# GAMES-UChile/mogptk

Hardware: AMD Instinct MI355X
Metric: log-marginal-likelihood+grad evals/sec, MOSM C=4 N=8192; 1/2/4/8 GPU (higher is better)
Workload: dtype f64

## Files before the change

include/mogp_hip.h:

```cpp
#ifndef MOGP_HIP_H
#define MOGP_HIP_H

#include <stdint.h>

#ifdef __cplusplus
extern "C" {
#endif

#define MOGP_OK            0
#define MOGP_EINVAL       -1
#define MOGP_EHIP         -2
#define MOGP_ENOTPD       -3
#define MOGP_ENONFINITE   -4
#define MOGP_ENODEVICE    -5

#define MOGP_TERM_WIDTH(D) (2 + 3 * (D))
#define MOGP_MOMENT_WIDTH(D) (2 + 3 * (D))

typedef struct mogp_ctx mogp_ctx;
typedef struct mogp_model mogp_model;

const char* mogp_version(void);
const char* mogp_last_error(void);
int  mogp_device_count(void);
// ... 108 lines not shown
int  mogp_model_fetch(mogp_model* m, int which, double* out);

int  mogp_snelson_eval(mogp_model* m, int64_t M, const double* Z, const double* noise_var, double jitter, const double* kff_diag, int flags,
                       double* lml, double* mom_uu, double* mom_uf, double* gZ, double* trGA, double* hsum, double* jitter_abs, int64_t* info);
int  mogp_snelson_predict(mogp_model* m, int64_t M, const double* Z, const double* noise_var, double jitter, const double* kff_diag,
                          const double* kss_diag, int64_t S, const double* Xs, double* mu, double* var, int64_t* info);
int  mogp_snelson_eval_sharded(mogp_model* m, int64_t M, const double* Z, const double* noise_var, double jitter, const double* kff_diag,
                               int flags, double* lml, double* mom_uu, double* mom_uf, double* gZ, double* trGA, double* hsum,
                               double* jitter_abs, int64_t* info);
int  mogp_snelson_predict_sharded(mogp_model* m, int64_t M, const double* Z, const double* noise_var, double jitter, const double* kff_diag,
                                  const double* kss_diag, int64_t S, const double* Xs, double* mu, double* var, int64_t* info);

int  mogp_svgp_forward(mogp_model* m, int64_t M, const double* Z, const double* q_mu, const double* q_sqrt, double jitter,
                       const double* kff_diag, int dense, int64_t S, const double* Xs, const double* kss_diag,
                       double* mu, double* var, double* jitter_abs, int64_t* info);
int  mogp_svgp_backward(mogp_model* m, const double* e, const double* f, double* mom_uu, double* mom_uf, double* gZ, double* trGA,
                        double* g_qmu, double* g_qsqrt);
int  mogp_svgp_backward_sharded(mogp_model* m, const double* e, const double* f, double* mom_uu, double* mom_uf, double* gZ, double* trGA,
                                double* g_qmu, double* g_qsqrt);

int  mogp_oa_forward(mogp_model* m, const double* q_nu, const double* q_lambda, double* mu, double* var, double* kl, int64_t* info);
int  mogp_oa_backward(mogp_model* m, const double* e, const double* f, double* moments, double* g_nu, double* g_lambda);
int  mogp_oa_predict(mogp_model* m, const double* q_nu, const double* q_lambda, const double* kss_diag, int64_t S, const double* Xs,
                     int full, double* mu, double* var, int64_t* info);

int  mogp_sparse_predict_cov(mogp_model* m, int64_t S, double* cov);

int  mogp_mosm_terms(int C, int Q, int D, const double* w, const double* mu, const double* v, const double* th, const double* ph,
                     double twopi, double phase_scale, double* table);
int  mogp_mosm_terms_backward(int C, int Q, int D, const double* w, const double* mu, const double* v, const double* th, const double* ph,
                              double twopi, double phase_scale, const double* gtable, double* gw, double* gmu, double* gv, double* gth,
                              double* gph);

#ifdef __cplusplus
}
#endif
#endif
```

mogptk_amd/_lib.py:

```python
import atexit
import ctypes
import os
import threading
import weakref
import numpy as np

_HERE = os.path.dirname(os.path.abspath(__file__))
LIB_PATH = os.environ.get("MOGP_LIB_PATH") or os.path.join(_HERE, "csrc", "libmogp_hip.so")

MOGP_OK, MOGP_EINVAL, MOGP_EHIP, MOGP_ENOTPD, MOGP_ENONFINITE, MOGP_ENODEVICE = 0, -1, -2, -3, -4, -5
MOGP_EVAL_GRAD = 1
COMM_ID_BYTES = 128
ALLGATHER_CB = ctypes.CFUNCTYPE(ctypes.c_int, ctypes.c_void_p, ctypes.c_void_p, ctypes.c_void_p, ctypes.c_int64)
ALLREDUCE_CB = ctypes.CFUNCTYPE(ctypes.c_int, ctypes.c_void_p, ctypes.c_void_p, ctypes.c_int64)
ST_GRAM, ST_POTRF, ST_TRTRI, ST_LAUUM, ST_SOLVE, ST_MOMENTS, ST_TOTAL, ST_GEMM_KERNEL, ST_GRAM_KERNEL, ST_MOMENT_KERNEL, ST_COUNT = range(11)

_lib = None
_lock = threading.RLock()
_ctx = {}
_live = weakref.WeakSet()

c_dp = ctypes.POINTER(ctypes.c_double)
c_i64p = ctypes.POINTER(ctypes.c_int64)
c_ip = ctypes.POINTER(ctypes.c_int)
# ... 60 lines not shown
    "mogp_shard_alpha": (ctypes.c_int, [ctypes.c_void_p, ctypes.POINTER(ctypes.c_void_p), c_i64p]),
    "mogp_shard_finish": (ctypes.c_int, [ctypes.c_void_p, c_dp, c_dp, c_dp, c_i64p]),
    "mogp_dev_copy": (ctypes.c_int, [ctypes.c_void_p, ctypes.c_void_p, ctypes.c_int64, ctypes.c_int]),
    "mogp_set_profiling": (ctypes.c_int, [ctypes.c_void_p, ctypes.c_int]),
    "mogp_stage_ms": (ctypes.c_int, [ctypes.c_void_p, c_dp, c_i64p, c_dp]),
    "mogp_model_fetch": (ctypes.c_int, [ctypes.c_void_p, ctypes.c_int, c_dp]),
    "mogp_model_schedule": (ctypes.c_int, [ctypes.c_void_p, ctypes.POINTER(ctypes.c_int)]),
    "mogp_model_flow_replay": (ctypes.c_int, [ctypes.c_void_p, ctypes.c_int]),
    "mogp_model_flow_diag": (ctypes.c_int, [ctypes.c_void_p, ctypes.POINTER(ctypes.c_uint)]),
    "mogp_flow_plan": (ctypes.c_int, [ctypes.c_int, c_i64p, ctypes.c_int64, c_i64p]),
    "mogp_flow_plan_rhs": (ctypes.c_int, [ctypes.c_int, ctypes.c_int, c_i64p, ctypes.c_int64, ctypes.POINTER(ctypes.c_int64)]),
    "mogp_flow_trace": (ctypes.c_int, [ctypes.c_void_p, c_i64p, ctypes.c_int64, c_i64p]),
    "mogp_snelson_eval": (ctypes.c_int, [ctypes.c_void_p, ctypes.c_int64, c_dp, c_dp, ctypes.c_double, c_dp, ctypes.c_int,
                                         ctypes.POINTER(ctypes.c_double), c_dp, c_dp, c_dp, ctypes.POINTER(ctypes.c_double), c_dp,
                                         ctypes.POINTER(ctypes.c_double), c_i64p]),
    "mogp_snelson_predict": (ctypes.c_int, [ctypes.c_void_p, ctypes.c_int64, c_dp, c_dp, ctypes.c_double, c_dp, c_dp, ctypes.c_int64, c_dp,
                                            c_dp, c_dp, c_i64p]),
    "mogp_snelson_eval_sharded": (ctypes.c_int, [ctypes.c_void_p, ctypes.c_int64, c_dp, c_dp, ctypes.c_double, c_dp, ctypes.c_int,
                                         ctypes.POINTER(ctypes.c_double), c_dp, c_dp, c_dp, ctypes.POINTER(ctypes.c_double), c_dp,
                                         ctypes.POINTER(ctypes.c_double), c_i64p]),
    "mogp_snelson_predict_sharded": (ctypes.c_int, [ctypes.c_void_p, ctypes.c_int64, c_dp, c_dp, ctypes.c_double, c_dp, c_dp, ctypes.c_int64, c_dp,
                                            c_dp, c_dp, c_i64p]),
    "mogp_svgp_forward": (ctypes.c_int, [ctypes.c_void_p, ctypes.c_int64, c_dp, c_dp, c_dp, ctypes.c_double, c_dp, ctypes.c_int, ctypes.c_int64,
                                         c_dp, c_dp, c_dp, c_dp, ctypes.POINTER(ctypes.c_double), c_i64p]),
    "mogp_svgp_backward": (ctypes.c_int, [ctypes.c_void_p, c_dp, c_dp, c_dp, c_dp, c_dp, ctypes.POINTER(ctypes.c_double), c_dp, c_dp]),
    "mogp_svgp_backward_sharded": (ctypes.c_int, [ctypes.c_void_p, c_dp, c_dp, c_dp, c_dp, c_dp, ctypes.POINTER(ctypes.c_double), c_dp, c_dp]),
    "mogp_oa_forward": (ctypes.c_int, [ctypes.c_void_p, c_dp, c_dp, c_dp, c_dp, ctypes.POINTER(ctypes.c_double), c_i64p]),
    "mogp_oa_backward": (ctypes.c_int, [ctypes.c_void_p, c_dp, c_dp, c_dp, c_dp, c_dp]),
    "mogp_oa_predict": (ctypes.c_int, [ctypes.c_void_p, c_dp, c_dp, c_dp, ctypes.c_int64, c_dp, ctypes.c_int, c_dp, c_dp, c_i64p]),
    "mogp_sparse_predict_cov": (ctypes.c_int, [ctypes.c_void_p, ctypes.c_int64, c_dp]),
    "mogp_mosm_terms": (ctypes.c_int, [ctypes.c_int, ctypes.c_int, ctypes.c_int, c_dp, c_dp, c_dp, c_dp, c_dp, ctypes.c_double, ctypes.c_double, c_dp]),
    "mogp_mosm_terms_backward": (ctypes.c_int, [ctypes.c_int, ctypes.c_int, ctypes.c_int, c_dp, c_dp, c_dp, c_dp, c_dp, ctypes.c_double,
                                                ctypes.c_double, c_dp, c_dp, c_dp, c_dp, c_dp, c_dp]),
}


class MogpError(RuntimeError):
    def __init__(self, code, message, info=0):
        super().__init__(message)
        self.code = code
        self.info = info


def lib():
    global _lib
    with _lock:
        if _lib is None:
            if not os.path.exists(LIB_PATH):
                raise ImportError(
                    "libmogp_hip.so not found at %s: build it with `python __graft_entry__.py` "
                    "(hipcc --offload-arch=gfx950).  mogptk_amd has no CPU fallback." % LIB_PATH)
            l = ctypes.CDLL(LIB_PATH)
            for name, (res, args) in SIGNATURES.items():
                fn = getattr(l, name)
                fn.restype = res
                fn.argtypes = args
            _lib = l
    return _lib


def _dp(a):
    return None if a is None else a.ctypes.data_as(c_dp)


def _f64(a):
    return None if a is None else np.ascontiguousarray(a, dtype=np.float64)
# ... 40 lines not shown
    M2 = M1 if X2 is None else X2.shape[0]
    out = np.empty((M1, M2), dtype=np.float64)
    if kind is not None:
        kind = np.ascontiguousarray(kind, dtype=np.int32)
        shape = _f64(shape)
        assert kind.shape == table.shape[:3] and shape.shape == table.shape[:3]
        check(lib().mogp_gram_kinds(context(device), C, D, T, int(table.shape[3]), _dp(table), _ip(kind), _dp(shape), M1, _dp(X1),
                                    0 if X2 is None else M2, _dp(X2), _dp(out)))
        return out
    check(lib().mogp_gram_ex(context(device), C, D, T, int(table.shape[3]), _dp(table), M1, _dp(X1),
                             0 if X2 is None else M2, _dp(X2), _dp(out)))
    return out


def shutdown():
    with _lock:
        for h in list(_live):
            try:
                h.close()
            except Exception:
                pass
        if _lib is not None:
            for c in list(_ctx.values()):
                try:
                    _lib.mogp_ctx_destroy(c)
                except Exception:
                    pass
        _ctx.clear()


atexit.register(shutdown)


class ExactHandle:

    def __init__(self, device, X, y, C):
        X = _f64(X)
        y = _f64(np.asarray(y).reshape(-1))
        self.N = X.shape[0]
        self.D = X.shape[1] - 1
        self.C = C
        self.device = device
        h = ctypes.c_void_p()
        self._h = ctypes.c_void_p()
        check(lib().mogp_model_create(context(device), self.N, self.D, C, _dp(X), _dp(y), ctypes.byref(h)))
        self._h = h
        _live.add(self)

    def close(self):
        if getattr(self, "_h", None) is not None and self._h.value is not None:
            lib().mogp_model_destroy(self._h)
            self._h = ctypes.c_void_p()

    def __del__(self):
        try:
            self.close()
        except Exception:
            pass

    def set_y(self, y):
        y = _f64(np.asarray(y).reshape(-1))
        check(lib().mogp_model_set_y(self._h, _dp(y)))

    def set_mean(self, coef):
        if coef is None:
            check(lib().mogp_model_set_mean(self._h, None))
# ... 13 lines not shown
        self.T = table.shape[2]
        self.W = int(table.shape[3])
        check(lib().mogp_model_set_terms_ex(self._h, self.T, self.W, _dp(table)))

    def set_kinds(self, kind, shape):
        if kind is None:
            check(lib().mogp_model_set_kinds(self._h, self.T, None, None))
            return
        kind = np.ascontiguousarray(kind, dtype=np.int32)
        shape = _f64(shape)
        assert kind.shape == (self.C, self.C, self.T) and shape.shape == kind.shape
        check(lib().mogp_model_set_kinds(self._h, self.T, _ip(kind), _dp(shape)))

    def set_point_diag(self, kdiag):
        check(lib().mogp_model_set_point_diag(self._h, _dp(_f64(kdiag))))

    def eval(self, noise_var, jitter, grad=True, data_var=None):
        noise_var = _f64(noise_var)
        data_var = _f64(data_var)
        from .gpr.config import config as _cfg
        comm = getattr(_cfg, "comm", None)
        if grad and comm is not None and (comm.world > 1 or comm.force):
            if getattr(comm, "native", False):
                return self.eval_sharded(noise_var, jitter, data_var)
            from . import dist as _dist
            return _dist.sharded_eval(self, comm, noise_var, jitter, data_var)
        lml, trG, jit, info = ctypes.c_double(), ctypes.c_double(), ctypes.c_double(), ctypes.c_int64(0)
        moments, diagG = self._grad_outputs(grad)
        code = lib().mogp_exact_eval(self._h, _dp(noise_var), _dp(data_var), float(jitter),
                                     MOGP_EVAL_GRAD if grad else 0, ctypes.byref(lml), _dp(moments), _dp(diagG),
                                     ctypes.byref(trG), ctypes.byref(jit), ctypes.byref(info))
        check(code, info.value)
        return dict(lml=lml.value, moments=moments, diagG=diagG, trG=trG.value, jitter_abs=jit.value)

    def _grad_outputs(self, grad=True):
        C = self.C
        return (np.zeros((C * (C + 1) // 2, self.T, self.W)), np.zeros(C)) if grad else (None, None)

    def _held_out(self, key, entry, noise_var, jitter, grad, data_var, *score_args):
        noise_var = _f64(noise_var)
        data_var = _f64(data_var)
        score, trG, jit, info = ctypes.c_double(), ctypes.c_double(), ctypes.c_double(), ctypes.c_int64(0)
        mu, var = np.empty(self.N), np.empty(self.N)
        moments, diagG = self._grad_outputs(grad)
        code = entry(self._h, _dp(noise_var), _dp(data_var), float(jitter), MOGP_EVAL_GRAD if grad else 0, *score_args, ctypes.byref(score),
                     _dp(mu), _dp(var), _dp(moments), _dp(diagG), ctypes.byref(trG), ctypes.byref(jit), ctypes.byref(info))
        check(code, info.value)
        return {key: score.value, "mu": mu, "var": var, "moments": moments, "diagG": diagG, "trG": trG.value, "jitter_abs": jit.value}

    def loo(self, noise_var, jitter, grad=True, data_var=None):
        return self._held_out("loo", lib().mogp_exact_loo, noise_var, jitter, grad, data_var)

    def cv(self, noise_var, jitter, fold, nfolds, grad=True, data_var=None):
        fold = np.ascontiguousarray(fold, dtype=np.int32)
        if fold.shape != (self.N,):
            raise ValueError("fold must hold one label per training point")
        return self._held_out("cv", lib().mogp_exact_cv, noise_var, jitter, grad, data_var, fold.ctypes.data_as(ctypes.POINTER(ctypes.c_int32)), int(nfolds))

    def loo_bytes(self):
        b = ctypes.c_int64(0)
        check(lib().mogp_model_loo_bytes(self._h, ctypes.byref(b)))
        return int(b.value)

    def eval_sharded(self, noise_var, jitter, data_var=None):
        lml, trG, jit, info = ctypes.c_double(), ctypes.c_double(), ctypes.c_double(), ctypes.c_int64(0)
        moments, diagG = self._grad_outputs()
# ... 252 lines not shown
```

mogptk_amd/gpr/config.py:

```python
import numpy as np


class Config:
    dtype = np.float64
    device = 0
    positive_minimum = 1e-8
    comm = None
    accurate_fallback = True


config = Config()


def use_double_precision():
    config.dtype = np.float64


def use_single_precision():
    config.dtype = np.float32


def use_half_precision():
    raise NotImplementedError("half precision is not on the MI355X exact-GP path")


def use_gpu(n=None):
    from .._lib import lib
    count = lib().mogp_device_count()
    if count <= 0:
        print("HIP device is not available")
    elif n is not None and (not isinstance(n, int) or n < 0 or count <= n):
        print("HIP GPU '%s' is not available" % (n,))
    else:
        config.device = 0 if n is None else n


def use_hip(n=None):
    use_gpu(n)


def use_cpu(n=None):
# ... 17 lines not shown
```

mogptk_amd/gpr/model.py:

```python
import sys
import numpy as np
from contextlib import contextmanager
from math import erf, sqrt

from .config import config
from .parameter import Parameter, ParameterHolder
from .kernel import Kernel, MulKernel, ChangePointsKernel, terms_cache, KIND_TIMES, KIND_MASK, KIND_DOT, KIND_GATE, KIND_WDOT, group_diag_grad
from .likelihood import Likelihood, GaussianLikelihood
from .mean import Mean


class CholeskyException(Exception):

    def __init__(self, message, K, model):
        self.message = message
        self.K = K
        self.model = model

    def __str__(self):
        return self.message


def _to_array(X):
    if hasattr(X, "detach"):
        X = X.detach().cpu().numpy()
    return np.array(X, dtype=config.dtype)


def _leaf_kernels(kernel):
    subs = getattr(kernel, "kernels", None)
    if not subs or isinstance(kernel, (MulKernel, ChangePointsKernel)):
        return [kernel]
    return [leaf for k in subs for leaf in _leaf_kernels(k)]


def _enveloped(table, D):
    return table.shape[3] > 2 + 3 * D


def _channel_counts(Xk, C):
    return np.bincount(Xk[:, 0].astype(np.int64), minlength=C).astype(np.float64)


def _lml_constant(X):
    return 0.5 * X.shape[0] * np.log(2.0 * np.pi)


_PAIR_INDEX = {}


def _pair_index(C, lower):
    key = (C, lower)
    if key not in _PAIR_INDEX:
        _PAIR_INDEX[key] = np.tril_indices(C) if lower else tuple(np.divmod(np.arange(C * C), C))
    return _PAIR_INDEX[key]


def _gtable_from_moments(table, mom, D, lower=True, kind=None):
    C, T = table.shape[0], table.shape[2]
    gt = np.zeros((C, C, T, table.shape[3]))
    ii, jj = _pair_index(C, lower)
    tb = table[ii, jj]
    A = tb[..., 0]
    V = tb[..., 2:2 + D]
    M = tb[..., 2 + D:2 + 2 * D]
    m0, m4 = mom[..., 0], mom[..., 1]
    m1, m2, m3 = mom[..., 2:2 + D], mom[..., 2 + D:2 + 2 * D], mom[..., 2 + 2 * D:2 + 3 * D]
    g = np.empty_like(tb)
    g[..., 0] = m0
    g[..., 1] = -2.0 * np.pi * A * m4
    g[..., 2:2 + D] = -0.5 * A[..., None] * m1
    g[..., 2 + D:2 + 2 * D] = -2.0 * np.pi * A[..., None] * m3
    g[..., 2 + 2 * D:2 + 3 * D] = -V * A[..., None] * m2 - 2.0 * np.pi * M * (A * m4)[..., None]
    if tb.shape[-1] > 2 + 3 * D:
        Lv = tb[..., 2 + 3 * D:2 + 4 * D]
        g[..., 2 + 3 * D:2 + 4 * D] = -0.5 * A[..., None] * mom[..., 2 + 3 * D:2 + 4 * D]
        g[..., 2 + 4 * D:2 + 5 * D] = Lv * A[..., None] * mom[..., 2 + 4 * D:2 + 5 * D]
    if kind is not None:
# ... 368 lines not shown
                if np.any(taken):
                    raise ValueError("folds %d and %d overlap (point %d): folds are disjoint" % (labels[ind][taken][0], f, ind[taken][0]))
                labels[ind] = f
        if F == 0:
            raise ValueError("no folds: at least one point must be held out")
        sizes = np.bincount(labels[labels >= 0], minlength=F)
        for f in range(F):
            if sizes[f] == 0:
                raise ValueError("fold %d is empty" % f)
            if sizes[f] > self.FOLD_MAX:
                raise ValueError("fold %d holds %d points: the limit is %d points per fold, larger folds are not on the device"
                                 % (f, sizes[f], self.FOLD_MAX))
        return labels.astype(np.int32), F

    def _eval(self, grad, score="lml", folds=None):
        if score == "loo":
            self._refuse_sharded_loo()
        elif score == "cv":
            self._refuse_sharded_loo("leave-fold-out cross-validation")
            labels, F = self._fold_labels(folds)
        h, table, D = self._push_terms()
        with self._cholesky_guard():
            if score == "cv":
                run = lambda: h.cv(self._noise_var(), self.jitter, labels, F, grad=grad, data_var=self.data_variance)
            else:
                call = h.loo if score == "loo" else h.eval
                run = lambda: call(self._noise_var(), self.jitter, grad=grad, data_var=self.data_variance)
            res = run()
            again = self._check_conditioning(h, run) if grad or score != "lml" else None
            return (res if again is None else again), table, D

    CONDITION_WARN = 1e5

    def _check_conditioning(self, h, redo):
        if not hasattr(h, "condition_estimate"):
            return None
        est = h.condition_estimate()
        if est != est:
            return None
        accurate = getattr(h, "accurate_mode", False)
        if not accurate and est > self.CONDITION_WARN:
            fallback = getattr(config, "accurate_fallback", True) and hasattr(h, "set_accurate")
            if not getattr(self, "_cond_warned", False):
                self._cond_warned = True
                import warnings
                warnings.warn("the kernel matrix plus noise is ill-conditioned (cond >= %.1e from the Cholesky factor's diagonal): beyond ~1e6 - 1e7 the "
                              "fast schedules' LML and gradients leave a backward-stable factorisation's by more than 1e-9 / 1e-5 (at 1e8: ~1e-7 / ~1e-4); %s"
                              % (est, "evaluating in the backward-stable form from here on (about two and a half times slower)" if fallback
                                 else "a larger noise variance or jitter brings it back"), RuntimeWarning, stacklevel=5)
            if fallback:
                h.set_accurate(True)
                h.accurate_mode = True
                return redo()
        elif accurate and est < 0.1 * self.CONDITION_WARN:
            h.set_accurate(False)
            h.accurate_mode = False
        return None

    def log_marginal_likelihood(self):
        res, _, _ = self._eval(grad=False)
        return config.dtype(res["lml"])

    def _loss_impl(self, score="lml", folds=None):
        self.zero_grad(set_to_none=True)
        res, table, D = self._eval(grad=True, score=score, folds=folds)
        counts = self._train_counts()
        jit_rel = self.jitter * res["trG"] / self.X.shape[0]

        point_kinds = getattr(self._handle, "point_kinds", None)
        gt = _gtable_from_moments(table, res["moments"], D, lower=True, kind=point_kinds)
        if _enveloped(table, D) or point_kinds is not None:
            gt += jit_rel * self.kernel._point_diag_table_grad(table, self.kernel._kernel_format(self.X), D)
        else:
            kind = getattr(self._handle, "group_kinds", None)
            if kind is not None:
                for i in range(table.shape[0]):
                    gt[i, i, :, 0] += jit_rel * counts[i] * group_diag_grad(table[i, i, :, 0], kind[i, i])
            else:
                for i in range(table.shape[0]):
                    gt[i, i, :, 0] += jit_rel * counts[i]
        self.kernel._table_backward(-gt)

        self._noise_backward(res["diagG"] + jit_rel * counts)
        self._mean_backward(self._handle)
        return config.dtype(-res[score] - self.log_prior())

    def loo(self):
        res, _, _ = self._eval(grad=False, score="loo")
        return self._held_out(res)

    def _held_out(self, res):
        mu = res["mu"].reshape(-1, 1)
        if self.mean is not None and not (self._trainable_mean() and self._mean_affine()[0] is not None):
            mu = self._add_mean(mu, self.X)
        return mu.astype(config.dtype, copy=False), res["var"].reshape(-1, 1).astype(config.dtype, copy=False)

# ... 429 lines not shown
```

mogptk_amd/gpr/multioutput.py:

```python
import ctypes

import numpy as np

from .config import config
from .parameter import Parameter, _STRUCTURE_EPOCH
from .kernel import Kernel, MultiOutputKernel, term_width, cached_terms, KIND_TIMES, KIND_MASK, KIND_DOT, GROUP_MAX, group_slices

PI = np.pi


def _accumulate(p, gconstrained):
    p.accumulate_grad(gconstrained)


class IndependentMultiOutputKernel(MultiOutputKernel):

    def __init__(self, *kernels, output_dims=None):
        if output_dims is None:
            output_dims = len(kernels)
        super().__init__(output_dims)
        self.kernels = self._check_kernels(kernels, output_dims)
        self.input_dims = self.kernels[0].input_dims

    def __getitem__(self, key):
# ... 55 lines not shown
        super().__init__(output_dims, input_dims, active_dims)
        self.input_dims = input_dims
        self.weight = Parameter(np.ones((output_dims, Q)), lower=config.positive_minimum)
        self.mean = Parameter(np.zeros((output_dims, Q, input_dims)), lower=config.positive_minimum)
        self.variance = Parameter(np.ones((output_dims, Q, input_dims)), lower=config.positive_minimum)
        self.delay = Parameter(np.zeros((output_dims, Q, input_dims)))
        self.phase = Parameter(np.zeros((output_dims, Q)))
        if output_dims == 1:
            self.delay.train = False
            self.phase.train = False
        self.twopi = np.power(2.0 * np.pi, float(self.input_dims) / 2.0)

    _phase_scale = 1.0

    def _values(self):
        return self.weight(), self.mean(), self.variance(), self.delay(), self.phase()

    def _magnitude(self, w):
        return w[:, None] * w[None, :]

    def _amp_scale(self):
        return 1.0

    def _magnitude_backward(self, w, gmag):
        return np.sum(gmag * w[None, :], axis=1) + np.sum(gmag * w[:, None], axis=0)

    def _store(self, gw, gmu, gv, gth, gph):
        _accumulate(self.weight, gw)
        _accumulate(self.mean, gmu)
        _accumulate(self.variance, gv)
        if self.output_dims > 1:
            _accumulate(self.delay, gth)
            _accumulate(self.phase, gph)

    def _memo_key(self):
        parts = []
        for p in (self.weight, self.mean, self.variance, self.delay, self.phase):
            parts.append(p.data.tobytes())
            for b in (p.lower, p.upper):
                parts.append(b"-" if b is None else np.asarray(b, dtype=np.float64).tobytes())
            if p.pegged:
                parts.append(p.pegged_parameter.data.tobytes())
        return b"|".join(parts)

    def _pairs(self):
        key = self._memo_key()
        memo = self.__dict__.get("_pairs_memo")
        if memo is not None and memo[0] == key:
            return memo[1]
        out = self._pairs_compute()
        self.__dict__["_pairs_memo"] = (key, out)
        return out

    def _pairs_compute(self):
        w, mu, v, th, ph = self._values()
        vi, vj = v[:, None], v[None, :]
        mi, mj = mu[:, None], mu[None, :]
        s = vi + vj
        inv = 1.0 / s
        dmu = mi - mj
        return w, mu, v, th, ph, vi, vj, mi, mj, s, inv, dmu

    @cached_terms
    def _spectral_terms(self, D):
        if D != self.input_dims:
            raise ValueError("X must have %d input dimensions" % self.input_dims)
# ... 431 lines not shown
```

mogptk_amd/model.py:

```python
import os
import time
import math
import pickle
import inspect
import logging
import numpy as np

from . import gpr
from .dataset import DataSet
from .util import (mean_absolute_error, mean_absolute_percentage_error, symmetric_mean_absolute_percentage_error,
                   mean_squared_error, root_mean_squared_error)

logger = logging.getLogger("mogptk")


def LoadModel(filename, allow=None, trusted=False):
    filename += ".npy"
    with open(filename, "rb") as r:
        raw = r.read()
    from . import compat
    if compat.is_reference_checkpoint(raw):
        return compat.load_reference_model(raw)
    return compat.load_native_model(raw, allow=allow or (), trusted=trusted)

# ... 36 lines not shown
    def _build(self, kernel, x, y, y_err=None, mean=None):
        variance = self.variance
        if variance is None:
            variance = [1.0] * kernel.output_dims if kernel.output_dims is not None else 1.0
        return gpr.Snelson(kernel, x, y, Z=self.inducing_points, Z_init=self.init_inducing_points, variance=variance, jitter=self.jitter, mean=mean)


class OpperArchambeau:

    def __init__(self, likelihood=None, jitter=1e-6):
        self.likelihood = likelihood
        self.jitter = jitter

    def _build(self, kernel, x, y, y_err=None, mean=None):
        likelihood = self.likelihood if self.likelihood is not None else gpr.GaussianLikelihood(1.0)
        return gpr.OpperArchambeau(kernel, x, y, likelihood=likelihood, jitter=self.jitter, mean=mean)


class Hensman:

    def __init__(self, inducing_points=None, init_inducing_points="grid", likelihood=None, jitter=1e-6):
        self.inducing_points = inducing_points
        self.init_inducing_points = init_inducing_points
        self.likelihood = likelihood
        self.jitter = jitter

    def _build(self, kernel, x, y, y_err=None, mean=None):
        likelihood = self.likelihood if self.likelihood is not None else gpr.GaussianLikelihood(1.0)
        if self.inducing_points is None:
            return gpr.Hensman(kernel, x, y, likelihood=likelihood, jitter=self.jitter, mean=mean)
        return gpr.SparseHensman(kernel, x, y, Z=self.inducing_points, Z_init=self.init_inducing_points, likelihood=likelihood, jitter=self.jitter, mean=mean)


class _Adam:

    def __init__(self, params, lr=1e-3, betas=(0.9, 0.999), eps=1e-8, weight_decay=0.0, amsgrad=False, **unused):
        self.params = list(params)
        self.lr, self.betas, self.eps, self.wd, self.amsgrad = lr, betas, eps, weight_decay, amsgrad
        self.state = {}

    def step(self):
        b1, b2 = self.betas
        flat = [p for p in self.params if p.grad is not None and p.data.dtype == np.float64 and p.grad.dtype == np.float64]
        if len(flat) > 1:
            key = tuple(id(p) for p in flat)
            st = self.state.get("flat")
            if st is None or st["key"] != key:
                self._unflatten()
                parts = [self._tensor_state(p) for p in flat]
                st = dict(key=key, t=[q["t"] for q in parts], m=np.concatenate([q["m"].ravel() for q in parts]),
                          v=np.concatenate([q["v"].ravel() for q in parts]), vmax=np.concatenate([q["vmax"].ravel() for q in parts]),
                          ends=np.cumsum([p.data.size for p in flat]))
                self.state["flat"] = st
            g = np.concatenate([p.grad.ravel() for p in flat])
            x = np.concatenate([p.data.ravel() for p in flat])
            if self.wd != 0.0:
                g = g + self.wd * x
            st["t"] = [t + 1 for t in st["t"]]
            st["m"] = b1 * st["m"] + (1.0 - b1) * g
            st["v"] = b2 * st["v"] + (1.0 - b2) * g * g
            v = st["v"]
            if self.amsgrad:
                st["vmax"] = np.maximum(st["vmax"], v)
                v = st["vmax"]
            if len(set(st["t"])) == 1:
                bc1, bc2 = 1.0 - b1 ** st["t"][0], 1.0 - b2 ** st["t"][0]
                x = x - (self.lr / bc1) * st["m"] / (np.sqrt(v) / math.sqrt(bc2) + self.eps)
            else:
                sizes = np.diff(np.concatenate([[0], st["ends"]]))
                bc1 = np.repeat([1.0 - b1 ** t for t in st["t"]], sizes)
                bc2 = np.repeat([1.0 - b2 ** t for t in st["t"]], sizes)
                x = x - (self.lr / bc1) * st["m"] / (np.sqrt(v) / np.sqrt(bc2) + self.eps)
            lo = 0
            for p, hi in zip(flat, st["ends"]):
                p.data = x[lo:hi].reshape(p.data.shape)
                lo = hi
            done = set(key)
        else:
            self._unflatten()
            done = set()
        for p in self.params:
            if p.grad is None or id(p) in done:
                continue
            g = p.grad
            if self.wd != 0.0:
                g = g + self.wd * p.data
            st = self._tensor_state(p)
            st["t"] += 1
            st["m"] = b1 * st["m"] + (1.0 - b1) * g
            st["v"] = b2 * st["v"] + (1.0 - b2) * g * g
            bc1 = 1.0 - b1 ** st["t"]
            bc2 = 1.0 - b2 ** st["t"]
            v = st["v"]
            if self.amsgrad:
                st["vmax"] = np.maximum(st["vmax"], v)
                v = st["vmax"]
            denom = np.sqrt(v) / math.sqrt(bc2) + self.eps
            p.data = p.data - (self.lr / bc1) * st["m"] / denom

    def _tensor_state(self, p):
        self._unflatten(only=id(p))
        return self.state.setdefault(id(p), dict(t=0, m=np.zeros_like(p.data), v=np.zeros_like(p.data), vmax=np.zeros_like(p.data)))

    def _unflatten(self, only=None):
        st = self.state.get("flat")
        if st is None or (only is not None and only not in st["key"]):
            return
# ... 545 lines not shown
```

Before: 96.78.

## Move MOSM parameter transforms, term table, and Adam update into native host step

```diff
diff --git a/include/mogp_hip.h b/include/mogp_hip.h
--- a/include/mogp_hip.h
+++ b/include/mogp_hip.h
@@ -164,6 +164,22 @@
                               double twopi, double phase_scale, const double* gtable, double* gw, double* gmu, double* gv, double* gth,
                               double* gph);
 
+#define MOGP_TRANSFORM_IDENTITY 0
+#define MOGP_TRANSFORM_SOFTPLUS 1
+#define MOGP_TRANSFORM_SIGMOID  2
+int  mogp_mosm_step_forward(int C, int Q, int D, int nscale, const double* raw, const int* tkind, const double* lower, const double* upper,
+                            const double* beta, const double* threshold, const double* lp, const double* en, double twopi, double phase_scale,
+                            double* cons, double* dcons, double* table, double* noise_var);
+int  mogp_mosm_step_backward(int C, int Q, int D, int nscale, const double* cons, const double* dcons, const double* table, const double* moments,
+                             const double* diagG, double trG, double jitter, const double* counts, int64_t N, double twopi, double phase_scale,
+                             const int* trained, double* graw);
+int  mogp_exact_step(mogp_model* m, int C, int Q, int D, int nscale, const double* raw, const int* tkind, const double* lower, const double* upper,
+                     const double* beta, const double* threshold, const double* lp, const double* en, double twopi, double phase_scale,
+                     const double* data_var, double jitter, const double* counts, const int* trained, double* cons, double* dcons, double* table, double* noise_var, double* moments,
+                     double* diagG, double* out5, double* graw, int64_t* info);
+int  mogp_adam_step(int nseg, const int64_t* ends, double* x, const double* g, double* m, double* v, double* vmax, double lr, double beta1,
+                    double beta2, double eps, double weight_decay, int amsgrad, const double* bc1, const double* bc2);
+
 #ifdef __cplusplus
 }
 #endif
diff --git a/mogptk_amd/_lib.py b/mogptk_amd/_lib.py
--- a/mogptk_amd/_lib.py
+++ b/mogptk_amd/_lib.py
@@ -116,6 +116,13 @@
     "mogp_mosm_terms": (ctypes.c_int, [ctypes.c_int, ctypes.c_int, ctypes.c_int, c_dp, c_dp, c_dp, c_dp, c_dp, ctypes.c_double, ctypes.c_double, c_dp]),
     "mogp_mosm_terms_backward": (ctypes.c_int, [ctypes.c_int, ctypes.c_int, ctypes.c_int, c_dp, c_dp, c_dp, c_dp, c_dp, ctypes.c_double,
                                                 ctypes.c_double, c_dp, c_dp, c_dp, c_dp, c_dp, c_dp]),
+    "mogp_mosm_step_forward": (ctypes.c_int, [ctypes.c_int] * 4 + [c_dp, c_ip, c_dp, c_dp, c_dp, c_dp, c_dp, c_dp, ctypes.c_double, ctypes.c_double,
+                                              c_dp, c_dp, c_dp, c_dp]),
+    "mogp_mosm_step_backward": (ctypes.c_int, [ctypes.c_int] * 4 + [c_dp] * 5 + [ctypes.c_double, ctypes.c_double, c_dp, ctypes.c_int64,
+                                                                               ctypes.c_double, ctypes.c_double, c_ip, c_dp]),
+    "mogp_exact_step": (ctypes.c_int, [ctypes.c_void_p] + [ctypes.c_int] * 4 + [c_dp, c_ip, c_dp, c_dp, c_dp, c_dp, c_dp, c_dp, ctypes.c_double, ctypes.c_double,
+                                                                               c_dp, ctypes.c_double, c_dp, c_ip] + [c_dp] * 8 + [c_i64p]),
+    "mogp_adam_step": (ctypes.c_int, [ctypes.c_int, c_i64p] + [c_dp] * 5 + [ctypes.c_double] * 5 + [ctypes.c_int, c_dp, c_dp]),
 }
 
 
@@ -222,6 +229,111 @@
 atexit.register(shutdown)
 
 
+TRANSFORM_IDENTITY, TRANSFORM_SOFTPLUS, TRANSFORM_SIGMOID = 0, 1, 2
+
+
+def _check_host(code, name):
+    if code != MOGP_OK:
+        raise MogpError(code, "%s failed (%d): a bad argument -- shape, transform kind or null pointer" % (name, code))
+
+
+class StepPlan:
+
+    def __init__(self, C, Q, D, nscale, transforms, twopi, phase_scale, counts, N, trained):
+        self.C, self.Q, self.D, self.nscale, self.N = int(C), int(Q), int(D), int(nscale), int(N)
+        sizes = [C * Q, C * Q * D, C * Q * D, C * Q * D, C * Q, nscale]
+        self.ends = np.cumsum(sizes)
+        self.starts = self.ends - sizes
+        self._cuts = [0] + [int(e) for e in self.ends]
+        self._trained = [bool(t) for t in trained]
+        self.params = ()
+        n = int(self.ends[-1])
+        W = 2 + 3 * D
+        self.tkind = np.zeros(n, dtype=np.int32)
+        self.lower, self.upper, self.beta, self.threshold = np.zeros(n), np.zeros(n), np.zeros(n), np.zeros(n)
+        for (kind, lo, up, beta, thr), a, b in zip(transforms, self.starts, self.ends):
+            self.tkind[a:b] = kind
+            for dst, val in ((self.lower, lo), (self.upper, up), (self.beta, beta), (self.threshold, thr)):
+                dst[a:b] = 0.0 if val is None else np.asarray(val, dtype=np.float64).reshape(-1)
+        self.trained = np.ascontiguousarray(trained, dtype=np.int32)
+        self.counts = _f64(counts)
+        assert self.trained.shape == (6,) and self.counts.shape == (C,)
+        self.raw, self.cons, self.dcons, self.graw = np.zeros(n), np.zeros(n), np.zeros(n), np.zeros(n)
+        self._scale = np.where(self.tkind == TRANSFORM_SOFTPLUS, self.beta, np.where(self.tkind == TRANSFORM_SIGMOID, 1.0, 0.0))
+        self._cap = np.where(self.tkind == TRANSFORM_SOFTPLUS, self.threshold, np.inf)
+        self._z, self.lp, self.en = np.zeros(n), np.zeros(n), np.zeros(n)
+        self.table = np.zeros((C, C, Q, W))
+        self.noise_var = np.zeros(C)
+        self.moments = np.zeros((C * (C + 1) // 2, Q, W))
+        self.diagG = np.zeros(C)
+        self.out = np.zeros(5)
+        self.info = ctypes.c_int64(0)
+        self.twopi, self.phase_scale = float(twopi), float(phase_scale)
+        shape = (self.C, self.Q, self.D, self.nscale)
+        self._fwd = shape + (_dp(self.raw), _ip(self.tkind), _dp(self.lower), _dp(self.upper), _dp(self.beta), _dp(self.threshold), _dp(self.lp), _dp(self.en),
+                             self.twopi, self.phase_scale, _dp(self.cons), _dp(self.dcons), _dp(self.table), _dp(self.noise_var))
+        self._bwd_head = shape + (_dp(self.cons), _dp(self.dcons), _dp(self.table), _dp(self.moments), _dp(self.diagG))
+        self._bwd_tail = (_dp(self.counts), self.N, self.twopi, self.phase_scale, _ip(self.trained), _dp(self.graw))
+        self._step_args = None
+
+    def gather(self, tensors):
+        np.concatenate([t.reshape(-1) for t in tensors], out=self.raw)
+        self.transcendentals()
+
+    def transcendentals(self):
+        z, lp, en = self._z, self.lp, self.en
+        with np.errstate(over="ignore", invalid="ignore"):
+            np.multiply(self._scale, self.raw, out=z)
+            np.negative(z, out=en)
+            np.exp(en, out=en)
+            np.minimum(z, self._cap, out=z)
+            np.exp(z, out=lp)
+            np.log1p(lp, out=lp)
+
+    def block(self, flat, i, shape):
+        return flat[self._cuts[i]:self._cuts[i + 1]].reshape(shape)
+
+    def scatter_grad(self):
+        g = self.graw.copy()
+        cuts = self._cuts
+        for i, p in enumerate(self.params):
+            p.grad = g[cuts[i]:cuts[i + 1]].reshape(p.data.shape) if self._trained[i] else None
+
+    def forward(self):
+        _check_host(lib().mogp_mosm_step_forward(*self._fwd), "mogp_mosm_step_forward")
+
+    def backward(self, trG, jitter):
+        _check_host(lib().mogp_mosm_step_backward(*self._bwd_head, float(trG), float(jitter), *self._bwd_tail), "mogp_mosm_step_backward")
+
+    def step_args(self, jitter, data_var):
+        c = self._step_args
+        if c is None or c[0] != jitter or c[1] is not data_var:
+            dv = _f64(data_var)
+            c = self._step_args = (jitter, data_var, dv, self._fwd[:14] + (_dp(dv), float(jitter), _dp(self.counts), _ip(self.trained)) + self._fwd[14:] +
+                                   (_dp(self.moments), _dp(self.diagG), _dp(self.out), _dp(self.graw), ctypes.byref(self.info)))
+        return c[3]
+
+    def condition_estimate(self):
+        lo, hi = self.out[3], self.out[4]
+        return float((hi / lo) ** 2) if lo > 0.0 else float("nan")
+
+
+class AdamPlan:
+
+    def __init__(self, ends, m, v, vmax):
+        self.ends = np.ascontiguousarray(ends, dtype=np.int64)
+        n, k = int(self.ends[-1]), self.ends.shape[0]
+        for a in (m, v, vmax):
+            assert a.dtype == np.float64 and a.flags.c_contiguous and a.shape == (n,)
+        self.m, self.v, self.vmax = m, v, vmax
+        self.x, self.g, self.bc1, self.bc2 = np.empty(n), np.empty(n), np.empty(k), np.empty(k)
+        self._head = (k, self.ends.ctypes.data_as(c_i64p), _dp(self.x), _dp(self.g), _dp(m), _dp(v), _dp(vmax))
+        self._tail = (_dp(self.bc1), _dp(self.bc2))
+
+    def step(self, lr, beta1, beta2, eps, weight_decay, amsgrad):
+        _check_host(lib().mogp_adam_step(*self._head, lr, beta1, beta2, eps, weight_decay, 1 if amsgrad else 0, *self._tail), "mogp_adam_step")
+
+
 class ExactHandle:
 
     def __init__(self, device, X, y, C):
@@ -301,6 +413,12 @@
                                      ctypes.byref(trG), ctypes.byref(jit), ctypes.byref(info))
         check(code, info.value)
         return dict(lml=lml.value, moments=moments, diagG=diagG, trG=trG.value, jitter_abs=jit.value)
+
+    def step(self, plan, jitter, data_var=None):
+        assert plan.C == self.C and plan.D == self.D and plan.N == self.N
+        self.T, self.W = plan.Q, 2 + 3 * plan.D
+        code = lib().mogp_exact_step(self._h, *plan.step_args(jitter, data_var))
+        check(code, plan.info.value)
 
     def _grad_outputs(self, grad=True):
         C = self.C
diff --git a/mogptk_amd/csrc/hoststep.hip b/mogptk_amd/csrc/hoststep.hip
--- /dev/null
+++ b/mogptk_amd/csrc/hoststep.hip
@@ -0,0 +1,159 @@
+#include "../../include/mogp_hip.h"
+
+#include <cmath>
+#include <vector>
+
+#pragma clang fp contract(off)
+
+namespace {
+
+double numpy_sum(const double* a, int64_t n) {
+    if (n < 8) {
+        double r = -0.0;
+        for (int64_t i = 0; i < n; ++i) r += a[i];
+        return r;
+    }
+    if (n <= 128) {
+        double r[8];
+        for (int k = 0; k < 8; ++k) r[k] = a[k];
+        int64_t i = 8;
+        for (; i < n - (n % 8); i += 8)
+            for (int k = 0; k < 8; ++k) r[k] += a[i + k];
+        double res = ((r[0] + r[1]) + (r[2] + r[3])) + ((r[4] + r[5]) + (r[6] + r[7]));
+        for (; i < n; ++i) res += a[i];
+        return res;
+    }
+    int64_t n2 = n / 2;
+    n2 -= n2 % 8;
+    return numpy_sum(a, n2) + numpy_sum(a + n2, n - n2);
+}
+
+struct Blocks {
+    int64_t off[7];
+    Blocks(int C, int Q, int D, int nscale) {
+        const int64_t cq = (int64_t)C * Q, cqd = cq * D;
+        off[0] = 0; off[1] = cq; off[2] = off[1] + cqd; off[3] = off[2] + cqd; off[4] = off[3] + cqd; off[5] = off[4] + cq; off[6] = off[5] + nscale;
+    }
+};
+
+bool bad_shape(int C, int Q, int D, int nscale) { return C <= 0 || Q <= 0 || D <= 0 || (nscale != 1 && nscale != C); }
+
+}
+
+extern "C" {
+
+int mogp_mosm_step_forward(int C, int Q, int D, int nscale, const double* raw, const int* tkind, const double* lower, const double* upper,
+                           const double* beta, const double* threshold, const double* lp, const double* en, double twopi, double phase_scale,
+                           double* cons, double* dcons, double* table, double* noise_var) {
+    if ((lp == nullptr) != (en == nullptr)) return MOGP_EINVAL;
+    if (bad_shape(C, Q, D, nscale) || !raw || !tkind || !lower || !upper || !beta || !threshold || !cons || !dcons || !table || !noise_var)
+        return MOGP_EINVAL;
+    const Blocks b(C, Q, D, nscale);
+    const int64_t n = b.off[6];
+    for (int64_t k = 0; k < n; ++k) {
+        const double x = raw[k];
+        switch (tkind[k]) {
+        case MOGP_TRANSFORM_IDENTITY:
+            cons[k] = x; dcons[k] = 1.0;
+            break;
+        case MOGP_TRANSFORM_SOFTPLUS: {
+            const double z = beta[k] * x;
+            if (z > threshold[k]) { cons[k] = lower[k] + x; dcons[k] = 1.0; }
+            else { cons[k] = lower[k] + (lp ? lp[k] : std::log1p(std::exp(z))) / beta[k]; dcons[k] = 1.0 / (1.0 + (en ? en[k] : std::exp(-z))); }
+            break;
+        }
+        case MOGP_TRANSFORM_SIGMOID: {
+            const double s = 1.0 / (1.0 + (en ? en[k] : std::exp(-x))), span = upper[k] - lower[k];
+            cons[k] = lower[k] + span * s; dcons[k] = span * s * (1.0 - s);
+            break;
+        }
+        default:
+            return MOGP_EINVAL;
+        }
+    }
+    const int rc = mogp_mosm_terms(C, Q, D, cons + b.off[0], cons + b.off[1], cons + b.off[2], cons + b.off[3], cons + b.off[4], twopi, phase_scale, table);
+    if (rc != MOGP_OK) return rc;
+    for (int c = 0; c < C; ++c) {
+        const double s = cons[b.off[5] + (nscale == C ? c : 0)];
+        noise_var[c] = s * s;
+    }
+    return MOGP_OK;
+}
+
+int mogp_mosm_step_backward(int C, int Q, int D, int nscale, const double* cons, const double* dcons, const double* table, const double* moments,
+                            const double* diagG, double trG, double jitter, const double* counts, int64_t N, double twopi, double phase_scale,
+                            const int* trained, double* graw) {
+    if (bad_shape(C, Q, D, nscale) || N <= 0 || !cons || !dcons || !table || !moments || !diagG || !counts || !trained || !graw) return MOGP_EINVAL;
+    const Blocks b(C, Q, D, nscale);
+    const int W = 2 + 3 * D;
+    const double jit_rel = jitter * trG / (double)N;
+    const double m2pi = -2.0 * M_PI, p2pi = 2.0 * M_PI;
+
+    std::vector<double> gt((size_t)C * C * Q * W, 0.0);
+    for (int i = 0; i < C; ++i)
+        for (int j = 0; j <= i; ++j)
+            for (int q = 0; q < Q; ++q) {
+                const int64_t at = (((int64_t)i * C + j) * Q + q) * W;
+                const double* tb = table + at;
+                const double* mo = moments + (((int64_t)i * (i + 1) / 2 + j) * Q + q) * W;
+                double* g = gt.data() + at;
+                const double A = tb[0], m0 = mo[0], m4 = mo[1];
+                g[0] = m0;
+                g[1] = m2pi * A * m4;
+                for (int d = 0; d < D; ++d) {
+                    const double V = tb[2 + d], M = tb[2 + D + d], m1 = mo[2 + d], m2 = mo[2 + D + d], m3 = mo[2 + 2 * D + d];
+                    g[2 + d] = -0.5 * A * m1;
+                    g[2 + D + d] = m2pi * A * m3;
+                    g[2 + 2 * D + d] = -V * A * m2 - p2pi * M * (A * m4);
+                }
+                if (i == j) g[0] += jit_rel * counts[i];
+            }
+    for (double& x : gt) x = -x;
+
+    const int64_t cq = (int64_t)C * Q, cqd = cq * D;
+    std::vector<double> gc(2 * cq + 3 * cqd);
+    double* gw = gc.data(), *gmu = gw + cq, *gv = gmu + cqd, *gth = gv + cqd, *gph = gth + cqd;
+    const int rc = mogp_mosm_terms_backward(C, Q, D, cons + b.off[0], cons + b.off[1], cons + b.off[2], cons + b.off[3], cons + b.off[4], twopi,
+                                            phase_scale, gt.data(), gw, gmu, gv, gth, gph);
+    if (rc != MOGP_OK) return rc;
+    for (int blk = 0; blk < 5; ++blk) {
+        if (!trained[blk]) continue;
+        for (int64_t k = b.off[blk]; k < b.off[blk + 1]; ++k) graw[k] = gc[k] * dcons[k];
+    }
+    if (trained[5]) {
+        std::vector<double> gvar(C);
+        for (int c = 0; c < C; ++c) gvar[c] = diagG[c] + jit_rel * counts[c];
+        const int64_t o = b.off[5];
+        if (nscale == C && C > 1)
+            for (int c = 0; c < C; ++c) graw[o + c] = -(2.0 * cons[o + c] * gvar[c]) * dcons[o + c];
+        else
+            graw[o] = -(2.0 * cons[o] * numpy_sum(gvar.data(), C)) * dcons[o];
+    }
+    return MOGP_OK;
+}
+
+int mogp_adam_step(int nseg, const int64_t* ends, double* x, const double* g, double* m, double* v, double* vmax, double lr, double beta1,
+                   double beta2, double eps, double weight_decay, int amsgrad, const double* bc1, const double* bc2) {
+    if (nseg < 0 || !ends || !x || !g || !m || !v || !bc1 || !bc2 || (amsgrad && !vmax)) return MOGP_EINVAL;
+    const double c1 = 1.0 - beta1, c2 = 1.0 - beta2;
+    int64_t k = 0;
+    for (int s = 0; s < nseg; ++s) {
+        if (ends[s] < k) return MOGP_EINVAL;
+        const double step = lr / bc1[s], root2 = std::sqrt(bc2[s]);
+        for (; k < ends[s]; ++k) {
+            double gk = g[k];
+            if (weight_decay != 0.0) gk = gk + weight_decay * x[k];
+            m[k] = beta1 * m[k] + c1 * gk;
+            v[k] = beta2 * v[k] + c2 * gk * gk;
+            double vk = v[k];
+            if (amsgrad) {
+                if (!(vmax[k] >= vk)) vmax[k] = (vmax[k] != vmax[k]) ? vmax[k] : vk;
+                vk = vmax[k];
+            }
+            x[k] = x[k] - step * m[k] / (std::sqrt(vk) / root2 + eps);
+        }
+    }
+    return MOGP_OK;
+}
+
+}
diff --git a/mogptk_amd/csrc/step.hip b/mogptk_amd/csrc/step.hip
--- /dev/null
+++ b/mogptk_amd/csrc/step.hip
@@ -0,0 +1,27 @@
+#include "mogp_model.h"
+
+using namespace mogp;
+
+extern "C" {
+
+int mogp_exact_step(mogp_model* m, int C, int Q, int D, int nscale, const double* raw, const int* tkind, const double* lower, const double* upper,
+                    const double* beta, const double* threshold, const double* lp, const double* en, double twopi, double phase_scale,
+                    const double* data_var, double jitter,
+                    const double* counts, const int* trained, double* cons, double* dcons, double* table, double* noise_var, double* moments,
+                    double* diagG, double* out5, double* graw, int64_t* info) {
+    if (!m || !out5) return fail(MOGP_EINVAL, "mogp_exact_step: null argument");
+    if (C != m->C || D != m->D) return fail(MOGP_EINVAL, "mogp_exact_step: C and D must be the model's");
+    int rc;
+    if ((rc = mogp_mosm_step_forward(C, Q, D, nscale, raw, tkind, lower, upper, beta, threshold, lp, en, twopi, phase_scale, cons, dcons, table, noise_var)))
+        return fail(rc, "mogp_exact_step: bad argument (forward)");
+    if ((rc = mogp_model_set_terms(m, Q, table))) return rc;
+    double lml = 0.0, trG = 0.0, jit = 0.0;
+    if ((rc = mogp_exact_eval(m, noise_var, data_var, jitter, MOGP_EVAL_GRAD, &lml, moments, diagG, &trG, &jit, info))) return rc;
+    out5[0] = lml; out5[1] = trG; out5[2] = jit;
+    out5[3] = m->pivot_min; out5[4] = m->pivot_max;
+    if ((rc = mogp_mosm_step_backward(C, Q, D, nscale, cons, dcons, table, moments, diagG, trG, jitter, counts, m->N, twopi, phase_scale, trained, graw)))
+        return fail(rc, "mogp_exact_step: bad argument (backward)");
+    return MOGP_OK;
+}
+
+}
diff --git a/mogptk_amd/gpr/config.py b/mogptk_amd/gpr/config.py
--- a/mogptk_amd/gpr/config.py
+++ b/mogptk_amd/gpr/config.py
@@ -1,3 +1,5 @@
+from os import environ as _environ
+
 import numpy as np
 
 
@@ -7,6 +9,7 @@
     positive_minimum = 1e-8
     comm = None
     accurate_fallback = True
+    host_fast = _environ.get("MOGP_HOST_FAST", "1") != "0"
 
 
 config = Config()
diff --git a/mogptk_amd/gpr/model.py b/mogptk_amd/gpr/model.py
--- a/mogptk_amd/gpr/model.py
+++ b/mogptk_amd/gpr/model.py
@@ -4,10 +4,11 @@
 from math import erf, sqrt
 
 from .config import config
-from .parameter import Parameter, ParameterHolder
+from .parameter import Parameter, ParameterHolder, Softplus, Sigmoid, _STRUCTURE_EPOCH
 from .kernel import Kernel, MulKernel, ChangePointsKernel, terms_cache, KIND_TIMES, KIND_MASK, KIND_DOT, KIND_GATE, KIND_WDOT, group_diag_grad
 from .likelihood import Likelihood, GaussianLikelihood
 from .mean import Mean
+from .multioutput import MultiOutputSpectralMixtureKernel
 
 
 class CholeskyException(Exception):
@@ -44,6 +45,15 @@
 
 def _lml_constant(X):
     return 0.5 * X.shape[0] * np.log(2.0 * np.pi)
+
+
+_F64 = np.dtype(np.float64)
+_STEP_KINDS = {type(None): 0, Softplus: 1, Sigmoid: 2}
+
+
+def _step_signature(p):
+    t = p.transform
+    return (type(t), t, getattr(t, "lower", None), getattr(t, "upper", None), getattr(t, "beta", None), getattr(t, "threshold", None), p.data.shape)
 
 
 _PAIR_INDEX = {}
@@ -478,10 +488,11 @@
 
     CONDITION_WARN = 1e5
 
-    def _check_conditioning(self, h, redo):
-        if not hasattr(h, "condition_estimate"):
-            return None
-        est = h.condition_estimate()
+    def _check_conditioning(self, h, redo, est=None):
+        if est is None:
+            if not hasattr(h, "condition_estimate"):
+                return None
+            est = h.condition_estimate()
         if est != est:
             return None
         accurate = getattr(h, "accurate_mode", False)
@@ -507,7 +518,67 @@
         res, _, _ = self._eval(grad=False)
         return config.dtype(res["lml"])
 
+    def _step_plan(self, score):
+        k = self.kernel
+        if (score != "lml" or not getattr(config, "host_fast", True) or config.dtype != np.float64 or getattr(config, "comm", None) is not None
+                or type(k) is not MultiOutputSpectralMixtureKernel or self.mean is not None or type(self.likelihood) is not GaussianLikelihood):
+            return None
+        h = self._device_handle()
+        plan = getattr(h, "_step_plan", None)
+        if plan is not None and plan.kernel is k and plan.likelihood is self.likelihood and plan.X is self.X and plan.epoch == _STRUCTURE_EPOCH[0]:
+            for p, s in zip(plan.params, plan.sigs):
+                t = p.transform
+                if (t is not s[1] or p.pegged_parameter is not None or p.prior is not None or p.data.shape != s[6] or (p.data.dtype is not _F64 and p.data.dtype != _F64)
+                        or (t is not None and (t.lower is not s[2] or getattr(t, "upper", None) is not s[3] or getattr(t, "beta", None) != s[4]
+                                               or getattr(t, "threshold", None) != s[5]))):
+                    break
+            else:
+                return plan
+        return self._new_step_plan(h)
+
+    def _new_step_plan(self, h):
+        k = self.kernel
+        if not hasattr(h, "step") or getattr(h, "radial_kinds", False) or getattr(h, "point_diag_set", False):
+            return None
+        blocks, trained = k._step_blocks()
+        params = blocks + (self.likelihood.scale,)
+        epoch = _STRUCTURE_EPOCH[0]
+        plist = self._parameter_list()
+        if len(plist) != len(params):
+            return None
+        for p, q in zip(plist, params):
+            if p is not q or p.pegged_parameter is not None or p.prior is not None or p.data.dtype != np.float64:
+                return None
+        sigs = [_step_signature(p) for p in params]
+        C, D, Q = k.output_dims, k.input_dims, k.weight.shape[1]
+        scale = params[5]
+        shapes = [(C, Q), (C, Q, D), (C, Q, D), (C, Q, D), (C, Q), scale.shape]
+        if D != self._D or scale.shape not in ((), (C,)) or any(s[6] != shape for s, shape in zip(sigs, shapes)) or any(s[0] not in _STEP_KINDS for s in sigs):
+            return None
+        from .._lib import StepPlan
+        plan = StepPlan(C, Q, D, scale.data.size, [(_STEP_KINDS[s[0]],) + s[2:6] for s in sigs], k.twopi, k._phase_scale, self._train_counts(),
+                        self.X.shape[0], trained + (True,))
+        plan.params, plan.sigs, plan.X, plan.kernel, plan.likelihood, plan.epoch = params, sigs, self.X, k, self.likelihood, epoch
+        h._step_plan = plan
+        h.radial_kinds, h.group_kinds, h.point_kinds = False, None, None
+        return plan
+
+    def _loss_native(self, plan):
+        h = self._handle
+        for p in plan.params:
+            p.grad = None
+        plan.gather([p.data for p in plan.params])
+        run = lambda: h.step(plan, self.jitter, self.data_variance)
+        with self._cholesky_guard():
+            run()
+            self._check_conditioning(h, run, plan.condition_estimate())
+        plan.scatter_grad()
+        return config.dtype(-plan.out[0])
+
     def _loss_impl(self, score="lml", folds=None):
+        plan = self._step_plan(score)
+        if plan is not None:
+            return self._loss_native(plan)
         self.zero_grad(set_to_none=True)
         res, table, D = self._eval(grad=True, score=score, folds=folds)
         counts = self._train_counts()
diff --git a/mogptk_amd/gpr/multioutput.py b/mogptk_amd/gpr/multioutput.py
--- a/mogptk_amd/gpr/multioutput.py
+++ b/mogptk_amd/gpr/multioutput.py
@@ -111,6 +111,10 @@
         if self.output_dims > 1:
             _accumulate(self.delay, gth)
             _accumulate(self.phase, gph)
+
+    def _step_blocks(self):
+        multi = self.output_dims > 1
+        return (self.weight, self.mean, self.variance, self.delay, self.phase), (True, True, True, multi, multi)
 
     def _memo_key(self):
         parts = []
diff --git a/mogptk_amd/model.py b/mogptk_amd/model.py
--- a/mogptk_amd/model.py
+++ b/mogptk_amd/model.py
@@ -92,16 +92,21 @@
         return gpr.SparseHensman(kernel, x, y, Z=self.inducing_points, Z_init=self.init_inducing_points, likelihood=likelihood, jitter=self.jitter, mean=mean)
 
 
+_F64 = np.dtype(np.float64)
+
+
 class _Adam:
 
     def __init__(self, params, lr=1e-3, betas=(0.9, 0.999), eps=1e-8, weight_decay=0.0, amsgrad=False, **unused):
         self.params = list(params)
         self.lr, self.betas, self.eps, self.wd, self.amsgrad = lr, betas, eps, weight_decay, amsgrad
         self.state = {}
+        self._native = None
 
     def step(self):
         b1, b2 = self.betas
-        flat = [p for p in self.params if p.grad is not None and p.data.dtype == np.float64 and p.grad.dtype == np.float64]
+        f64 = _F64
+        flat = [p for p in self.params if p.grad is not None and (p.data.dtype is f64 or p.data.dtype == f64) and (p.grad.dtype is f64 or p.grad.dtype == f64)]
         if len(flat) > 1:
             key = tuple(id(p) for p in flat)
             st = self.state.get("flat")
@@ -112,27 +117,43 @@
                           v=np.concatenate([q["v"].ravel() for q in parts]), vmax=np.concatenate([q["vmax"].ravel() for q in parts]),
                           ends=np.cumsum([p.data.size for p in flat]))
                 self.state["flat"] = st
-            g = np.concatenate([p.grad.ravel() for p in flat])
-            x = np.concatenate([p.data.ravel() for p in flat])
-            if self.wd != 0.0:
-                g = g + self.wd * x
-            st["t"] = [t + 1 for t in st["t"]]
-            st["m"] = b1 * st["m"] + (1.0 - b1) * g
-            st["v"] = b2 * st["v"] + (1.0 - b2) * g * g
-            v = st["v"]
-            if self.amsgrad:
-                st["vmax"] = np.maximum(st["vmax"], v)
-                v = st["vmax"]
-            if len(set(st["t"])) == 1:
-                bc1, bc2 = 1.0 - b1 ** st["t"][0], 1.0 - b2 ** st["t"][0]
-                x = x - (self.lr / bc1) * st["m"] / (np.sqrt(v) / math.sqrt(bc2) + self.eps)
-            else:
-                sizes = np.diff(np.concatenate([[0], st["ends"]]))
-                bc1 = np.repeat([1.0 - b1 ** t for t in st["t"]], sizes)
-                bc2 = np.repeat([1.0 - b2 ** t for t in st["t"]], sizes)
-                x = x - (self.lr / bc1) * st["m"] / (np.sqrt(v) / np.sqrt(bc2) + self.eps)
+            st["t"] = ts = [t + 1 for t in st["t"]]
+            if gpr.config.host_fast:
+                plan = self._native
+                if plan is None or plan.m is not st["m"] or plan.v is not st["v"] or plan.vmax is not st["vmax"]:
+                    from . import _lib
+                    plan = self._native = _lib.AdamPlan(st["ends"], st["m"], st["v"], st["vmax"])
+                np.concatenate([p.grad.ravel() for p in flat], out=plan.g)
+                np.concatenate([p.data.ravel() for p in flat], out=plan.x)
+                if ts.count(ts[0]) == len(ts):
+                    plan.bc1.fill(1.0 - b1 ** ts[0])
+                    plan.bc2.fill(1.0 - b2 ** ts[0])
+                else:
+                    plan.bc1[:] = [1.0 - b1 ** t for t in ts]
+                    plan.bc2[:] = [1.0 - b2 ** t for t in ts]
+                plan.step(self.lr, b1, b2, self.eps, self.wd, self.amsgrad)
+                x = plan.x.copy()
+            else:
+                g = np.concatenate([p.grad.ravel() for p in flat])
+                x = np.concatenate([p.data.ravel() for p in flat])
+                if self.wd != 0.0:
+                    g = g + self.wd * x
+                st["m"] = b1 * st["m"] + (1.0 - b1) * g
+                st["v"] = b2 * st["v"] + (1.0 - b2) * g * g
+                v = st["v"]
+                if self.amsgrad:
+                    st["vmax"] = np.maximum(st["vmax"], v)
+                    v = st["vmax"]
+                if len(set(st["t"])) == 1:
+                    bc1, bc2 = 1.0 - b1 ** st["t"][0], 1.0 - b2 ** st["t"][0]
+                    x = x - (self.lr / bc1) * st["m"] / (np.sqrt(v) / math.sqrt(bc2) + self.eps)
+                else:
+                    sizes = np.diff(np.concatenate([[0], st["ends"]]))
+                    bc1 = np.repeat([1.0 - b1 ** t for t in st["t"]], sizes)
+                    bc2 = np.repeat([1.0 - b2 ** t for t in st["t"]], sizes)
+                    x = x - (self.lr / bc1) * st["m"] / (np.sqrt(v) / np.sqrt(bc2) + self.eps)
             lo = 0
-            for p, hi in zip(flat, st["ends"]):
+            for p, hi in zip(flat, st["ends"].tolist()):
                 p.data = x[lo:hi].reshape(p.data.shape)
                 lo = hi
             done = set(key)
```

Result: faster. 98.38 (median of 6 runs) (+1.7%).
